# mungerct/Stabilized_Navier_Stokes_Flow_FEniCSx

Hardware: AMD Instinct MI355X
Metric: M-DOF/s (assembly+solve) per Newton iteration (higher is better)
Workload: dtype f64

## Files before the change

### stabilized_navier_stokes_flow_fenicsx_amd/csrc/sns_policy.h

```cpp
#pragma once
#include <algorithm>
#include <cmath>
#include <cstdint>
#include <vector>

#include "sns.h"

namespace sns {
namespace policy {

inline int coarsest_rows(const sns_options& o) { return std::max(o.amg_coarse_size, std::min(o.amg_dense_rows, 4096)); }
inline int small_inverse_rows(const sns_options& o) { return std::max(o.amg_coarse_size, 40); }
enum CoarsestKind { COARSEST_SMALL_INVERSE = 0, COARSEST_BLOCKED_INVERSE = 1, COARSEST_SWEEPS = 2 };
inline CoarsestKind coarsest_kind(const sns_options& o, int64_t rows) {
    if (rows <= small_inverse_rows(o)) return COARSEST_SMALL_INVERSE;
    if (rows <= o.amg_dense_rows) return COARSEST_BLOCKED_INVERSE;
    return COARSEST_SWEEPS;
}
inline bool replicate_from(const sns_options& o, int level, int64_t rows_global, bool fits) {
    return level >= 1 && o.amg_replicate_rows > 0 && rows_global <= (int64_t)o.amg_replicate_rows &&
           rows_global > (int64_t)small_inverse_rows(o) && fits;
}
constexpr int DISTRIBUTED_DENSE_MAX_DOFS = 640;
constexpr int GRAPH_MAX_ROWS = 150000;
// ... 236 lines not shown
enum AssemblyState { STATE_W = 0, STATE_GEXT = 1, STATE_SNAPPED = 2 };
struct AssemblyPlan {
    int error = SNS_OK;
    const char* message = "";
    AssemblyRoute route = ROUTE_STAGED;
    AssemblyState state = STATE_W;
    ElementKernel element = ELEMENT_NONE;
    bool bc_check = false, offdiag = false, diag = false, store_K = false, Fe_out = false, gather_matrix = false,
         gather_residual = false, lift = false, bc_residual = false, matrix = false;
};

inline AssemblyPlan plan_assembly(const AssemblyFacts& f, bool violated = true) {
    AssemblyPlan p;
    auto refuse = [&](const char* why) { p.error = SNS_E_ARG; p.message = why; return p; };
    if (f.form != SNS_FORM_STOKES && f.form != SNS_FORM_NS) return refuse("bad form");
    const bool ns = f.form == SNS_FORM_NS;
    if (ns && !f.has_w) return refuse("NS form needs a state vector");
    p.matrix = f.want_matrix;
    if (f.dim == 2) {
        if (!f.cells) return refuse("empty mesh");
        p.route = ns ? ROUTE_NS_2D : ROUTE_STOKES_2D;
        p.offdiag = f.want_matrix;
        p.diag = f.want_matrix || (!ns && f.has_F);
        if (ns) {
            p.bc_check = f.has_F;
            p.element = f.want_matrix ? ELEMENT_NONE : ELEMENT_RESIDUAL;
            p.Fe_out = p.gather_residual = !f.want_matrix;
            p.lift = f.has_F && violated;
        } else {
            p.state = f.has_w ? STATE_SNAPPED : STATE_GEXT;
            p.bc_residual = f.has_w && f.has_F;
        }
        return p;
    }
    const bool try_fused = f.want_matrix && f.fused && ns && f.cells && !f.variant;
    p.bc_check = ns && f.cells && ((!f.want_matrix && f.has_F) || try_fused);
    const bool fast_residual = p.bc_check && !violated && !f.variant;
    if (try_fused || (!ns && !f.has_w && f.want_matrix && f.fused && f.cells)) {
        p.route = ns ? ROUTE_FUSED_NS : ROUTE_FUSED_STOKES;
        p.state = ns ? STATE_W : STATE_GEXT;
        p.offdiag = p.diag = true;
        p.lift = ns && f.has_F && !fast_residual;
        return p;
    }
    p.element = fast_residual ? ELEMENT_RESIDUAL : f.cells ? ELEMENT_STAGED : ELEMENT_NONE;
    p.store_K = p.element == ELEMENT_STAGED && f.want_matrix;
    p.Fe_out = p.element == ELEMENT_RESIDUAL || (p.element == ELEMENT_STAGED && f.has_F);
    p.gather_matrix = f.want_matrix;
    p.gather_residual = f.has_F;
    return p;
}

struct HandleFacts {
    int dim = 3;
    bool partitioned = false, tt_on = false, vl_on = false, bf_on = false, ev_on = false;
    bool has_facets = false, traction_on = false, backflow_on = false;
};
enum FactBit {
    IS_NOT_3D = 1, IS_PARTITIONED = 2, HAS_TIME_TERM = 4, HAS_LAW = 8, HAS_FORCE = 16, HAS_FIELD = 32, NO_FACETS = 64, HAS_TRACTION = 128,
    HAS_BACKFLOW = 256, HAS_BOUNDARY_FLOW = HAS_TRACTION | HAS_BACKFLOW
};
enum Family { FAMILY_FORM = 0, FAMILY_BOUNDARY, FAMILY_STABILITY, FAMILY_STATE_GRADIENT, FAMILY_RAW_JACOBIAN };
enum FormRequest {
    REQ_SET_TIME_TERM = 0, REQ_CLEAR_TIME_TERM, REQ_SET_CARREAU, REQ_SET_NEWTONIAN, REQ_SET_FIELD ,
    REQ_TIME_STEP, REQ_SHAPE_GRADIENT, REQ_RECOVER_GRADIENT, REQ_ERROR_INDICATOR, REQ_SCALAR ,
    REQ_ELEMENT_VISCOSITY , REQ_FORM_VARIANT, REQ_COUNT
};
enum BoundaryRequest { BREQ_SET_FACETS = 0, BREQ_SET_FLOW, BREQ_SET_SCALAR, BREQ_COUNT };
enum StabilityRequest { SREQ_MASS_APPLY = 0, SREQ_ARNOLDI, SREQ_COUNT, SREQ_MASS_APPLY_TRANSPOSE = SREQ_COUNT, SREQ_ARNOLDI_LEFT, SREQ_KINDS };
constexpr int GREQ_STATE_GRADIENT = 0;
enum RawJacobianRequest { JREQ_APPLY = 0, JREQ_SET_DIRICHLET, JREQ_COUNT };
struct Verdict {
    int error = SNS_OK;
    const char* tail = "";
};
struct Rule {
    Family family;
    int request;
    unsigned any_of;
    int code;
    const char* tail;
};
constexpr Rule RULES[] = {
    {FAMILY_FORM, REQ_SET_TIME_TERM, IS_NOT_3D, SNS_E_ARG, "3-D handles only"},
    {FAMILY_FORM, REQ_SET_TIME_TERM, IS_PARTITIONED, SNS_E_STATE, "not with a communicator attached (partitioned time stepping is not built)"},
    {FAMILY_FORM, REQ_SET_TIME_TERM, HAS_LAW, SNS_E_STATE, "not with a viscosity law set (the transient form has no law)"},
    {FAMILY_FORM, REQ_CLEAR_TIME_TERM, IS_NOT_3D, SNS_E_ARG, "3-D handles only"},
    {FAMILY_FORM, REQ_CLEAR_TIME_TERM, IS_PARTITIONED, SNS_E_STATE, "not with a communicator attached (partitioned time stepping is not built)"},
    {FAMILY_FORM, REQ_SET_CARREAU, IS_NOT_3D, SNS_E_ARG, "3-D handles only"},
    {FAMILY_FORM, REQ_SET_CARREAU, IS_PARTITIONED, SNS_E_STATE, "not with a communicator attached (partitioned handles have no law)"},
    {FAMILY_FORM, REQ_SET_CARREAU, HAS_TIME_TERM, SNS_E_STATE, "not with a time term set (the transient form has no law)"},
    {FAMILY_FORM, REQ_SET_CARREAU, HAS_FORCE | HAS_FIELD, SNS_E_STATE, "not with a body force or a viscosity field set"},
    {FAMILY_FORM, REQ_SET_NEWTONIAN, IS_NOT_3D, SNS_E_ARG, "3-D handles only"},
    {FAMILY_FORM, REQ_SET_NEWTONIAN, IS_PARTITIONED, SNS_E_STATE, "not with a communicator attached (partitioned handles have no law)"},
    {FAMILY_FORM, REQ_SET_NEWTONIAN, HAS_TIME_TERM, SNS_E_STATE, "not with a time term set (the transient form has no law)"},
    {FAMILY_FORM, REQ_SET_FIELD, IS_NOT_3D, SNS_E_ARG, "3-D handles only"},
    {FAMILY_FORM, REQ_SET_FIELD, IS_PARTITIONED, SNS_E_STATE, "not with a communicator attached (partitioned handles have no external fields)"},
    {FAMILY_FORM, REQ_SET_FIELD, HAS_LAW, SNS_E_STATE, "not with a viscosity law set"},
    {FAMILY_FORM, REQ_TIME_STEP, IS_NOT_3D, SNS_E_ARG, "3-D handles only"},
    {FAMILY_FORM, REQ_TIME_STEP, IS_PARTITIONED, SNS_E_STATE, "not with a communicator attached (partitioned time stepping is not built)"},
    {FAMILY_FORM, REQ_TIME_STEP, HAS_LAW, SNS_E_STATE, "not with a viscosity law set (the transient form has no law)"},
    {FAMILY_FORM, REQ_SHAPE_GRADIENT, IS_PARTITIONED, SNS_E_STATE, "not with a communicator attached (partitioned shape gradients are not built)"},
    {FAMILY_FORM, REQ_SHAPE_GRADIENT, HAS_LAW, SNS_E_STATE, "not with a viscosity law set (the mesh derivative of nu_e is not built)"},
    {FAMILY_FORM, REQ_SHAPE_GRADIENT, HAS_FORCE | HAS_FIELD, SNS_E_STATE,
     "not with a body force or a viscosity field set (the mesh derivative is not built with them)"},
    {FAMILY_FORM, REQ_SHAPE_GRADIENT, HAS_BOUNDARY_FLOW, SNS_E_STATE,
     "not with a boundary traction or backflow term set (the mesh derivative of the facet terms is not built)"},
    {FAMILY_FORM, REQ_RECOVER_GRADIENT, IS_PARTITIONED, SNS_E_STATE, "not with a communicator attached (partitioned gradient recovery is not built)"},
    {FAMILY_FORM, REQ_ERROR_INDICATOR, IS_PARTITIONED, SNS_E_STATE,
     "not with a communicator attached (a partitioned indicator needs a halo exchange of G)"},
    {FAMILY_FORM, REQ_SCALAR, IS_NOT_3D, SNS_E_ARG, "3-D handles only"},
    {FAMILY_FORM, REQ_SCALAR, IS_PARTITIONED, SNS_E_STATE, "not with a communicator attached (partitioned scalar transport is not built)"},
    {FAMILY_FORM, REQ_ELEMENT_VISCOSITY, IS_NOT_3D, SNS_E_ARG, "3-D handles only"},
    {FAMILY_FORM, REQ_FORM_VARIANT, IS_NOT_3D, SNS_E_ARG, "3-D handles only"},

    {FAMILY_BOUNDARY, BREQ_SET_FACETS, IS_NOT_3D, SNS_E_ARG, "3-D handles only"},
    {FAMILY_BOUNDARY, BREQ_SET_FACETS, IS_PARTITIONED, SNS_E_STATE, "not with a communicator attached (partitioned boundary terms are not built)"},
    {FAMILY_BOUNDARY, BREQ_SET_FLOW, IS_NOT_3D, SNS_E_ARG, "3-D handles only"},
    {FAMILY_BOUNDARY, BREQ_SET_FLOW, IS_PARTITIONED, SNS_E_STATE, "not with a communicator attached (partitioned boundary terms are not built)"},
    {FAMILY_BOUNDARY, BREQ_SET_FLOW, NO_FACETS, SNS_E_STATE, "set the boundary facets first (sns_set_boundary_facets)"},
    {FAMILY_BOUNDARY, BREQ_SET_SCALAR, IS_NOT_3D, SNS_E_ARG, "3-D handles only"},
    {FAMILY_BOUNDARY, BREQ_SET_SCALAR, IS_PARTITIONED, SNS_E_STATE, "not with a communicator attached (partitioned boundary terms are not built)"},
    {FAMILY_BOUNDARY, BREQ_SET_SCALAR, NO_FACETS, SNS_E_STATE, "set the boundary facets first (sns_set_boundary_facets)"},

    {FAMILY_STABILITY, SREQ_MASS_APPLY, IS_NOT_3D, SNS_E_ARG, "3-D handles only"},
    {FAMILY_STABILITY, SREQ_MASS_APPLY, IS_PARTITIONED, SNS_E_STATE, "not with a communicator attached (partitioned stability analysis is not built)"},
    {FAMILY_STABILITY, SREQ_MASS_APPLY, HAS_LAW, SNS_E_STATE, "not with a viscosity law set (the mass operator of the law's form is not built)"},
    {FAMILY_STABILITY, SREQ_ARNOLDI, IS_NOT_3D, SNS_E_ARG, "3-D handles only"},
    {FAMILY_STABILITY, SREQ_ARNOLDI, IS_PARTITIONED, SNS_E_STATE, "not with a communicator attached (partitioned stability analysis is not built)"},
    {FAMILY_STABILITY, SREQ_ARNOLDI, HAS_LAW, SNS_E_STATE, "not with a viscosity law set (the mass operator of the law's form is not built)"},
    {FAMILY_STABILITY, SREQ_ARNOLDI, HAS_TIME_TERM, SNS_E_STATE, "not with a time term set (the analysis sets its own and clears it)"},

    {FAMILY_STATE_GRADIENT, GREQ_STATE_GRADIENT, IS_NOT_3D, SNS_E_ARG, "3-D handles only"},
    {FAMILY_STATE_GRADIENT, GREQ_STATE_GRADIENT, IS_PARTITIONED, SNS_E_STATE, "not with a communicator attached (the partitioned Hessian pass is not built)"},
    {FAMILY_STATE_GRADIENT, GREQ_STATE_GRADIENT, HAS_LAW, SNS_E_STATE, "not with a viscosity law set (the second derivative of nu_e is not built)"},
    {FAMILY_STATE_GRADIENT, GREQ_STATE_GRADIENT, HAS_TIME_TERM, SNS_E_STATE, "not with a time term set (the pass is taken on the steady form)"},
    {FAMILY_STATE_GRADIENT, GREQ_STATE_GRADIENT, HAS_FORCE, SNS_E_STATE,
     "not with a body force set (J depends on f through the stabilisation's weighting: that contraction is not built)"},
    {FAMILY_STATE_GRADIENT, GREQ_STATE_GRADIENT, HAS_BACKFLOW, SNS_E_STATE,
     "not with a backflow coefficient set (the Hessian of the backflow term is not built)"},

    {FAMILY_RAW_JACOBIAN, JREQ_APPLY, IS_PARTITIONED, SNS_E_STATE, "not with a communicator attached (the partitioned raw-Jacobian pass is not built)"},
    {FAMILY_RAW_JACOBIAN, JREQ_APPLY, HAS_BACKFLOW, SNS_E_STATE,
     "not with a backflow coefficient set (the backflow term's share of the raw Jacobian is not built)"},
    {FAMILY_RAW_JACOBIAN, JREQ_SET_DIRICHLET, IS_PARTITIONED, SNS_E_STATE,
     "not with a communicator attached (partitioned handles keep the Dirichlet values they were created with)"},
};

enum Rows { ROWS_ALL = 0, ROWS_ARG = SNS_E_ARG, ROWS_STATE = SNS_E_STATE };
inline Verdict check_request(Family family, int request, const HandleFacts& f, Rows rows = ROWS_ALL) {
    if (family == FAMILY_STABILITY && request >= SREQ_COUNT) request -= SREQ_COUNT;
    const unsigned facts = (f.dim != 3) * IS_NOT_3D | f.partitioned * IS_PARTITIONED | f.tt_on * HAS_TIME_TERM | f.vl_on * HAS_LAW |
                           f.bf_on * HAS_FORCE | f.ev_on * HAS_FIELD | (!f.has_facets) * NO_FACETS | f.traction_on * HAS_TRACTION |
                           f.backflow_on * HAS_BACKFLOW;
    for (const Rule& r : RULES)
        if (r.family == family && r.request == request && (facts & r.any_of))
            return (rows == ROWS_ALL || r.code == rows) ? Verdict{r.code, r.tail} : Verdict{};
    return {};
}
inline Verdict check_request(Family family, int request, const HandleFacts& f, const Verdict& arguments) {
    Verdict v = check_request(family, request, f, ROWS_ARG);
    if (v.error == SNS_OK) v = arguments;
    if (v.error == SNS_OK) v = check_request(family, request, f, ROWS_STATE);
    return v;
}

constexpr int STABILITY_M_MIN = 2, STABILITY_M_MAX = 64;
struct ArnoldiArgs {
    int m = STABILITY_M_MAX;
    double shift = 0.0, breakdown_rel = 1e-6;
};
inline Verdict check_arnoldi_args(const ArnoldiArgs& a) {
    if (a.m < STABILITY_M_MIN || a.m > STABILITY_M_MAX) return {SNS_E_ARG, "m must lie in [2, 64]"};
    if (!(a.shift >= 0.0) || !(a.shift <= 1.7976931348623157e308)) return {SNS_E_ARG, "the shift must be finite and >= 0"};
    if (!(a.breakdown_rel > 0.0) || !(a.breakdown_rel < 1.0)) return {SNS_E_ARG, "breakdown_rel must lie in (0, 1)"};
    return {};
}
inline Verdict check_arnoldi_extend_args(const ArnoldiArgs& a, int k) {
    const Verdict v = check_arnoldi_args(a);
    if (v.error != SNS_OK) return v;
    if (k < 1 || k > a.m - 1) return {SNS_E_ARG, "k must lie in [1, m - 1]"};
    return {};
}
inline Verdict check_state_gradient_args(double c_jac, double c_mass) {
    if (!(c_jac - c_jac == 0.0) || !(c_mass - c_mass == 0.0)) return {SNS_E_ARG, "the coefficients must be finite"};
    return {};
}

struct RawJacobianArgs {
    int form = SNS_FORM_NS;
    bool aliased = false, variant = false;
};
inline Verdict check_raw_jacobian_args(const RawJacobianArgs& a) {
    if (a.form == SNS_FORM_STOKES) return {SNS_E_ARG, "the Stokes forms are not supported"};
    if (a.form != SNS_FORM_NS) return {SNS_E_ARG, "bad form"};
    if (a.aliased) return {SNS_E_ARG, "x and y must not be the same vector"};
    if (a.variant) return {SNS_E_STATE, "not with a perturbed form variant set (the pass holds the reference's constants only)"};
    return {};
}

inline Verdict check_form_request(FormRequest request, const HandleFacts& f) { return check_request(FAMILY_FORM, request, f); }
inline Verdict check_boundary_request(BoundaryRequest request, const HandleFacts& f) { return check_request(FAMILY_BOUNDARY, request, f); }
inline Verdict check_stability_request(StabilityRequest request, const HandleFacts& f, const ArnoldiArgs& a = {}) {
    const bool arnoldi = request == SREQ_ARNOLDI || request == SREQ_ARNOLDI_LEFT;
    return check_request(FAMILY_STABILITY, request, f, arnoldi ? check_arnoldi_args(a) : Verdict{});
}
inline Verdict check_stability_extend_request(StabilityRequest request, const HandleFacts& f, const ArnoldiArgs& a, int k) {
    return check_request(FAMILY_STABILITY, request, f, check_arnoldi_extend_args(a, k));
}
inline Verdict check_state_gradient_request(const HandleFacts& f, double c_jac = 1.0, double c_mass = 0.0) {
    return check_request(FAMILY_STATE_GRADIENT, GREQ_STATE_GRADIENT, f, check_state_gradient_args(c_jac, c_mass));
}
inline Verdict check_raw_jacobian_request(RawJacobianRequest request, const HandleFacts& f, const RawJacobianArgs& a = {}) {
    return check_request(FAMILY_RAW_JACOBIAN, request, f, request == JREQ_APPLY ? check_raw_jacobian_args(a) : Verdict{});
}

struct FormKey {
    double sigma = 0.0, theta = 0.0;
    bool law_on = false;
    double lambda = 0.0, n = 1.0, r = 0.0;
    uint64_t nu_generation = 0;
    uint64_t boundary_generation = 0;
    bool operator==(const FormKey& o) const {
        return sigma == o.sigma && theta == o.theta && law_on == o.law_on && lambda == o.lambda && n == o.n && r == o.r &&
               nu_generation == o.nu_generation && boundary_generation == o.boundary_generation;
    }
};
struct OperatorKey {
    int form = -1;
    double reynolds = 0.0;
    bool transposed = false;
    FormKey f;
    double scalar[6] = {0, 0, 0, 0, 0, 0};
    bool operator==(const OperatorKey& o) const {
        return form == o.form && reynolds == o.reynolds && transposed == o.transposed && f == o.f &&
               std::equal(scalar, scalar + 6, o.scalar);
    }
};
inline void stamp_operator(OperatorKey& k, int form, double reynolds, const FormKey& f, const double* scalar_par = nullptr) {
    k.form = form;
    k.reynolds = reynolds;
    k.transposed = false;
    k.f = f;
    if (scalar_par) std::copy(scalar_par, scalar_par + 6, k.scalar);
}
inline bool new_operator(const OperatorKey& matrix, const OperatorKey& estimated, bool r3_estimates) {
    return !r3_estimates && !(matrix == estimated);
}

struct LevelDamping {
    double omega = 0.8, lambda_max = 0.0, omega_checked = 0.0, ritz_limit = 0.0;
};
constexpr int ESTIMATE_EVERY = 4;
constexpr double LAMBDA_CAP = 4.0 / 3.0;
constexpr int COMPOUNDING_SWEEPS = 3;
constexpr double GROWTH_BOUND = 0.9;
constexpr double GROWTH_STEP = GROWTH_BOUND;
constexpr int GROWTH_TRIALS = 6;
constexpr double RETRY_FACTOR = 0.7, RETRY_FLOOR = 0.4;

inline bool estimates_due(bool has_estimate, int pc_setups, bool new_operator) {
    return !has_estimate || pc_setups % ESTIMATE_EVERY == 0 || new_operator;
}
inline bool takes_growth_check(bool not_last, int sweeps_per_cycle) { return not_last && sweeps_per_cycle >= COMPOUNDING_SWEEPS; }
inline bool takes_ritz_limit(const sns_options& o, bool not_last, int sweeps_per_cycle) {
    return o.amg_ritz_limit && takes_growth_check(not_last, sweeps_per_cycle);
}
inline double capped_damping(double amg_omega, double backoff, double lambda_max, bool ritz, double ritz_limit) {
    double w = amg_omega * backoff;
    if (lambda_max > 0.0) w = std::min(amg_omega, LAMBDA_CAP / lambda_max) * backoff;
    if (ritz && ritz_limit > 0.0) w = std::min(w, ritz_limit * backoff);
    return w;
}
template <class Growth>
inline int checked_damping(double& w, Growth&& growth) {
    for (int trial = 0; trial < GROWTH_TRIALS; ++trial) {
        double g = 0.0;
        if (const int rc = growth(w, &g)) return rc;
        if (g < GROWTH_BOUND) break;
        w *= GROWTH_STEP;
    }
    return SNS_OK;
}
inline double held_damping(double w, double omega_checked) { return omega_checked > 0.0 ? std::min(w, omega_checked) : w; }
inline bool retryable(int reason) {
    return reason == SNS_KSP_DIVERGED_BREAKDOWN || reason == SNS_KSP_DIVERGED_NANORINF || reason == SNS_KSP_STALLED;
}
inline bool retry_offered(const sns_options& o, double backoff) {
    return o.pc_type == SNS_PC_AMG && o.amg_retry_damping != 0 && backoff > RETRY_FLOOR;
}
inline void back_off(double& backoff) { backoff *= RETRY_FACTOR; }
inline void back_off(LevelDamping& d) {
    d.omega *= RETRY_FACTOR;
    if (d.omega_checked > 0.0) d.omega_checked *= RETRY_FACTOR;
}
inline void forget_estimates(LevelDamping& d) { d.lambda_max = d.omega_checked = d.ritz_limit = 0.0; }

struct StepFacts {
    int nranks = 1, ksp_type = SNS_KSP_BICGSTAB, pc_type = SNS_PC_AMG;
    bool fine_plain_cycle = false, zero_guess_vouched = false, estimates_due = true, plain_step = false;
};
struct StepPlan {
    bool skip_zero_guess_residual = false, export_ax = false, staged_speculation = false, split_cycle = false,
         setup_two_streams = false;
    bool operator==(const StepPlan& o) const {
        return skip_zero_guess_residual == o.skip_zero_guess_residual && export_ax == o.export_ax &&
               staged_speculation == o.staged_speculation && split_cycle == o.split_cycle && setup_two_streams == o.setup_two_streams;
    }
};
inline StepPlan plan_step(const StepFacts& f) {
    StepPlan p;
    if (f.nranks != 1 || f.plain_step || f.ksp_type != SNS_KSP_BICGSTAB) return p;
    p.skip_zero_guess_residual = f.zero_guess_vouched;
    p.export_ax = true;
    p.split_cycle = f.pc_type == SNS_PC_AMG && f.fine_plain_cycle;
    p.staged_speculation = f.pc_type != SNS_PC_AMG || p.split_cycle;
    p.setup_two_streams = f.pc_type == SNS_PC_AMG && !f.estimates_due;
    return p;
}

}
}
```

### stabilized_navier_stokes_flow_fenicsx_amd/csrc/sns_setup.hip

```cpp
#include "sns_ctx.h"

namespace sns {

int alloc_level_vectors(Level& L) {
    const size_t nd = 4 * (size_t)L.n;
    SNS_TRY(L.x.alloc(nd));
    SNS_TRY(L.b.alloc(nd));
    SNS_TRY(L.r.alloc(nd));
    HIP_TRY(hipMemset(L.x, 0, nd * sizeof(double)));
    HIP_TRY(hipMemset(L.b, 0, nd * sizeof(double)));
    HIP_TRY(hipMemset(L.r, 0, nd * sizeof(double)));
    return SNS_OK;
}


int upload_pattern(Level& L, const HostPattern& P, hipStream_t s) {
    L.n = P.n;
    L.nnzb = P.nnzb;
    SNS_TRY(L.rowptr.upload(P.rowptr));
    SNS_TRY(L.colind.upload(P.colind));
    SNS_TRY(L.diag.upload(P.diag));
    SNS_TRY(L.vals.alloc((size_t)P.nnzb * 16));
    SNS_TRY(L.dinv.alloc((size_t)P.n * 16));
    SNS_TRY(L.slot_row.alloc((size_t)P.nnzb));
// ... 379 lines not shown
    const int per_rank_coarse = dist ? std::max(1, o.amg_coarse_size / h->comm->nranks) : o.amg_coarse_size;
    double flag[1] = {n_owned > per_rank_coarse ? 1.0 : 0.0};
    SNS_TRY(global_sum(h, flag, 1));
    more = flag[0] != 0.0 && !(!dist && l >= 1 && n_owned <= policy::coarsest_rows(o));
    return SNS_OK;
}

static int aggregate_level(sns_ctx* h, int l, const Front& f, std::vector<int32_t>& agg, int32_t& nc_owned, int64_t& nc_global,
                           bool& progress) {
    nc_owned = 0;
    if (l == 0 && h->opt.amg_aggregation >= 1) {
        SNS_TRY(aggregate_fine_by_strength(h, f.cur, f.points(), agg, nc_owned));
    } else {
        aggregate_nodes(f.cur, f.n_owned, agg_size(h->opt), agg, nc_owned, f.points());
    }
    if (l == 0) h->agg0 = agg;
    double prog[3] = {(double)f.n_owned, (double)nc_owned, (l == 0 && h->fine_rematched_local) ? 1.0 : 0.0};
    SNS_TRY(global_sum(h, prog, 3));
    if (l == 0) h->fine_rematched = prog[2] > 0.0;
    nc_global = (int64_t)prog[1];
    progress = !(prog[1] >= prog[0] || prog[1] == 0.0);
    if (l == 0 && progress) h->n_global_l1 = nc_global;
    return SNS_OK;
}

static int exchange_aggregate_ids(sns_ctx* h, int l, const Front& f, int32_t nc_owned, std::vector<int32_t>& agg, Plan& cplan,
                                  GhostIds& cghosts, int32_t& nc_total) {
    Comm* c = h->comm.get();
    Level& L = h->levels[l];
    std::vector<double> ids((size_t)4 * f.cur.n, -1.0);
    for (int32_t i = 0; i < f.n_owned; ++i) ids[(size_t)4 * i] = (double)agg[i];
    HIP_TRY(hipMemcpy(L.xg, ids.data(), ids.size() * sizeof(double), hipMemcpyHostToDevice));
    SNS_TRY(comm_exchange(c, c->plans[l], L.xg, h->stream));
    HIP_TRY(hipStreamSynchronize(h->stream));
    HIP_TRY(hipMemcpy(ids.data(), L.xg, ids.size() * sizeof(double), hipMemcpyDeviceToHost));
    HIP_TRY(hipMemset(L.xg, 0, ids.size() * sizeof(double)));
    std::vector<int32_t> owner_agg((size_t)f.cur.n);
    for (int32_t i = 0; i < f.cur.n; ++i) owner_agg[(size_t)i] = (int32_t)ids[(size_t)4 * i];
    return coarse_halo_lists(c->plans[l], owner_agg, nc_owned, agg, cplan, cghosts, nc_total);
}

static int attach_plan(sns_ctx* h, Plan& cplan, int level) {
    SNS_TRY(check_plan_symmetry(h, cplan, level));
    SNS_TRY(plan_upload(cplan));
    SNS_TRY(connect_plan(h, cplan));
    h->comm->plans.push_back(std::move(cplan));
    return SNS_OK;
}

static int flag_empty_aggregates(sns_ctx* h) {
    Level& L = h->levels[0];
    SNS_TRY(L.empty_c.alloc(4 * (size_t)std::max(1, L.nc)));
    if (L.nc > 0)
        hipLaunchKernelGGL(k_empty_coarse, dim3((unsigned)((4 * (int64_t)L.nc + 255) / 256)), dim3(256), 0, h->stream, L.nc, L.m_ptr,
                           L.m_idx, L.free_mask, L.empty_c);
    return SNS_OK;
}

int build_hierarchy(sns_ctx* h, const HostPattern& fine) {
    Comm* c = h->comm.get();
    const bool dist = c && c->active() && c->nranks > 1;
    Front f;
    SNS_TRY(start_front(h, fine, dist, f));
    for (int l = 0; l + 1 < h->opt.amg_max_levels; ++l) {
        bool replicate = false, more = false, progress = false;
        SNS_TRY(agree_replication(h, dist, l, f.n_owned, replicate));
        if (replicate) {
            SNS_TRY(build_replicated_tail(h, l, f));
            return plan_hierarchy(h);
        }
        SNS_TRY(agree_more_levels(h, dist, l, f.n_owned, more));
        if (!more) break;
        std::vector<int32_t> agg;
        int32_t nc_owned = 0;
        int64_t nc_global = 0;
        SNS_TRY(aggregate_level(h, l, f, agg, nc_owned, nc_global, progress));
        if (!progress) break;
        int32_t nc_total = nc_owned;
        Plan cplan;
        GhostIds cghosts;
        if (dist) SNS_TRY(exchange_aggregate_ids(h, l, f, nc_owned, agg, cplan, cghosts, nc_total));
        HostAggregation A;
        build_coarse_from_agg(f.cur, f.n_owned, agg, nc_owned, nc_total, A);
        SNS_TRY(add_next_level(h, l, f, A, nc_global, !dist || l == 0 || c->windows(), dist));
        if (dist) SNS_TRY(attach_plan(h, cplan, l + 1));
        if (l == 0) SNS_TRY(flag_empty_aggregates(h));
        advance(f, A, std::move(cghosts));
    }
    Level& last = h->levels.back();
    if (h->levels.size() > 1) SNS_TRY(dist ? alloc_distributed_coarsest_solver(h, last, f.ghosts) : alloc_coarsest_solver(h, last));
    h->tm.amg_levels = (int)h->levels.size();
    return plan_hierarchy(h);
}


int plan_hierarchy(sns_ctx* h) {
    const Comm* c = h->comm.get();
    const int nl = (int)h->levels.size();
    policy::Facts& f = h->facts;
    f = policy::Facts();
    f.nranks = (c && c->active()) ? std::max(1, c->nranks) : 1;
    f.rep_level = h->rep_level;
    f.rows_global_l1 = h->n_global_l1;
    f.windows = c && c->windows();
    f.team_overlap = h->team_overlap;
    f.fuse_puts = std::getenv("SNS_NO_CARRIED_PUT") == nullptr;
    const Level& last = h->levels.back();
    f.last = last.dense_gj ? policy::COARSEST_BLOCKED_INVERSE
                           : (last.dense_inv || h->cg_N > 0) ? policy::COARSEST_SMALL_INVERSE : policy::COARSEST_SWEEPS;
    f.rep_gather_fits = h->rep_level > 0 && c && c->peer && h->levels[h->rep_level].n_blk > 0 &&
                        (size_t)4 * h->rep_maxn * (size_t)c->nranks <= c->peer->ag_doubles;
    std::vector<double> mine((size_t)2 * nl + 1), all;
    mine[(size_t)2 * nl] = h->fine_rematched_local ? 1.0 : 0.0;
    for (int l = 0; l < nl; ++l) {
        const Level& L = h->levels[l];
        f.rows.push_back(L.n_global);
        f.has_blocks.push_back(L.blk_rows != nullptr);
        f.has_ap.push_back(L.ap_rowptr != nullptr);
        f.has_ap_rep.push_back(L.ap_colind_rep != nullptr);
        const bool wc = c && (size_t)l < c->plans.size() && c->plans[l].identity_recv && c->plans[l].win_recv[0] != nullptr;
        mine[(size_t)l] = wc ? 1.0 : 0.0;
        mine[(size_t)nl + l] = (double)L.n_owned;
    }
    if (f.nranks > 1) SNS_TRY(host_allgather(h, mine, all));
    else all = mine;
    f.win_capable.assign((size_t)nl, 1);
    f.max_owned.assign((size_t)nl, 0);
    for (size_t r = 0; r < all.size() / mine.size(); ++r) {
        if (all[r * mine.size() + 2 * (size_t)nl] != 0.0) f.fine_rematched = true;
        for (int l = 0; l < nl; ++l) {
            if (all[r * mine.size() + l] == 0.0) f.win_capable[(size_t)l] = 0;
            f.max_owned[(size_t)l] = std::max(f.max_owned[(size_t)l], (int64_t)all[r * mine.size() + nl + l]);
        }
    }
    h->plan = policy::plan_cycle(h->opt, f);
    return SNS_OK;
}


static int refresh_replicated_source(sns_ctx* h, const Level& L) {
    Level& C = h->levels[h->rep_level];
    if (L.nnzb > 0)
        HIP_TRY(hipMemcpyAsync(h->rep_vsend, L.vals, (size_t)L.nnzb * 16 * sizeof(double), hipMemcpyDeviceToDevice, h->stream));
    SNS_TRY(comm_allgather(h->comm.get(), h->rep_vsend, h->rep_vrecv, (int)(h->rep_maxnz * 16), h->stream));
    const int64_t nsrc = h->rep_maxnz * h->comm->nranks;
    hipLaunchKernelGGL(k_scatter_blocks, dim3((unsigned)((nsrc * 8 + 255) / 256)), dim3(256), 0, h->stream, nsrc, h->rep_valmap,
                       h->rep_vrecv, C.vals);
    return SNS_OK;
}

static int refresh_smoother_inverses(sns_ctx* h, const policy::LevelPlan& P, Level& L) {
    const int32_t rows = L.n_owned;
    if (rows > 0) hipLaunchKernelGGL(k_dinv, dim3((rows + 255) / 256), dim3(256), 0, h->stream, rows, L.diag, L.vals, L.dinv);
    if (!P.blocks) return SNS_OK;
    const int bf = h->opt.amg_f32_matrix == 2 ? 2 : 1;
    if (!L.binv32 || L.binv_fmt != bf) {
        SNS_TRY(L.binv32.alloc(binv_bytes_per_block(bf) * (size_t)std::max(1, L.n_blk)));
        L.binv_fmt = bf;
    }
    if (L.n_blk > 0)
        with_fmt(bf, [&](auto F) {
            hipLaunchKernelGGL((k_binv<F>), dim3((unsigned)((L.n_blk + 7) / 8)), dim3(256), 0, h->stream, L.n_blk, L.blk_rows,
                               L.blk_of, L.rowptr, L.colind, L.vals, L.binv32, h->d_sing);
        });
    return SNS_OK;
}

static int refresh_low_precision_copies(sns_ctx* h, const policy::LevelPlan& P, Level& L, bool not_last) {
    if (P.lp_fmt == 0) return SNS_OK;
    const int32_t rows = L.n_owned;
    if (!L.dinv32) SNS_TRY(L.dinv32.alloc((size_t)16 * std::max(1, L.n)));
    if (rows > 0)
        hipLaunchKernelGGL(k_cvt_f32, dim3(vec_grid(16 * (int64_t)rows)), dim3(256), 0, h->stream, 16 * (int64_t)rows, L.dinv,
                           L.dinv32);
    if (h->opt.amg_f32_matrix == 2) {
        if (!L.vals16) {
            SNS_TRY(L.vals16.alloc(std::max<size_t>(1, (size_t)L.nnzb * 4) * sizeof(uint2)));
            SNS_TRY(L.scale16.alloc((size_t)4 * std::max(1, L.n)));
        }
        const bool with_m = not_last && L.ap_rowptr && L.ap_nib && h->opt.amg_fused_post;
        if (with_m && !L.ap_vals16) {
            SNS_TRY(L.ap_vals16.alloc(std::max<size_t>(1, (size_t)L.ap_nnz * 4) * sizeof(uint2)));
            SNS_TRY(L.ap_scale16.alloc((size_t)4 * std::max(1, L.n)));
        }
        if (rows > 0) {
            const unsigned grid = (unsigned)((rows + 31) / 32);
            if (with_m)
                hipLaunchKernelGGL((k_lp_copies16<1>), dim3(grid), dim3(128), 0, h->stream, rows, L.rowptr, L.vals,
                                   (uint2*)L.vals16.get(), L.scale16, L.ap_rowptr, L.ap_colind, L.ap_ptr, L.ap_idx, L.ap_nib, L.agg,
                                   L.free_mask, (uint2*)L.ap_vals16.get(), L.ap_scale16);
            else
                hipLaunchKernelGGL((k_lp_copies16<0>), dim3(grid), dim3(128), 0, h->stream, rows, L.rowptr, L.vals,
                                   (uint2*)L.vals16.get(), L.scale16, (const int32_t*)nullptr, (const int32_t*)nullptr,
                                   (const int32_t*)nullptr, (const int32_t*)nullptr, (const uint64_t*)nullptr,
                                   (const int32_t*)nullptr, (const uint8_t*)nullptr, (uint2*)nullptr, (float*)nullptr);
        }
    }
    if (h->opt.amg_f32_matrix != 2) {
        if (!L.vals32) SNS_TRY(L.vals32.alloc((size_t)L.nnzb * 16));
        if (L.nnzb > 0)
            hipLaunchKernelGGL(k_cvt_f32, dim3(vec_grid(L.nnzb * 16)), dim3(256), 0, h->stream, L.nnzb * 16, L.vals, L.vals32);
    }
    return SNS_OK;
}

static int refresh_ap32(sns_ctx* h, const policy::LevelPlan& P, Level& L) {
    if (!(L.ap_rowptr && h->opt.amg_fused_post && P.lp_fmt == 1)) return SNS_OK;
    const int32_t rows = L.n_owned;
    if (!L.ap_vals32) SNS_TRY(L.ap_vals32.alloc((size_t)L.ap_nnz * 16));
    if (rows > 0)
        hipLaunchKernelGGL(k_ap_cvt32, dim3((unsigned)((4 * (int64_t)rows + 255) / 256)), dim3(256), 0, h->stream, rows,
                           L.ap_rowptr, L.ap_colind, L.ap_ptr, L.ap_idx, L.vals, L.agg, L.free_mask, (float4*)L.ap_vals32.get());
    return SNS_OK;
}

static void refresh_galerkin(sns_ctx* h, int l) {
    const Level& L = h->levels[l];
    Level& C = h->levels[l + 1];
    const int64_t nth = C.nnzb * 8;
    hipLaunchKernelGGL(k_galerkin, dim3((unsigned)((nth + 255) / 256)), dim3(256), 0, h->stream, C.nnzb, L.r_ptr, L.r_idx, L.vals,
                       C.slot_row, C.colind, (l == 0) ? L.empty_c.get() : (const uint8_t*)nullptr, L.m_ptr, C.vals);
}

static int refresh_coarsest_solver(sns_ctx* h, int l) {
    Level& L = h->levels[l];
    if (h->cg_N > 0) {
        const int N = h->cg_N, mr = 4 * h->cg_maxn;
        HIP_TRY(hipMemsetAsync(h->cg_rows, 0, (size_t)mr * N * sizeof(double), h->stream));
        const int64_t nth = L.nnzb * 16;
        if (nth > 0)
            hipLaunchKernelGGL(k_bsr_to_dense_map, dim3((unsigned)((nth + 255) / 256)), dim3(256), 0, h->stream, L.n_owned,
                               L.rowptr, L.colind, L.vals, h->cg_colmap, N, h->cg_rows);
        hipLaunchKernelGGL(k_pad_identity, dim3(1), dim3(256), 0, h->stream, 4 * L.n_owned, mr, h->comm->rank * mr, N, h->cg_rows);
        SNS_TRY(comm_allgather(h->comm.get(), h->cg_rows, h->cg_full, mr * N, h->stream));
        hipLaunchKernelGGL(k_dense_inverse, dim3(1), dim3(1024), 0, h->stream, N, h->cg_full, h->d_piv, h->d_sing);
    } else if (L.dense_gj) {
        const int N = 4 * L.n, Np = L.dense_np;
        HIP_TRY(hipMemsetAsync(L.dense_gj, 0, (size_t)Np * Np * sizeof(double), h->stream));
        const int64_t nth = L.nnzb * 16;
        hipLaunchKernelGGL(k_bsr_to_dense_ld, dim3((unsigned)((nth + 255) / 256)), dim3(256), 0, h->stream, L.nnzb, L.slot_row,
                           L.colind, L.vals, Np, L.dense_gj);
        if (Np > N) hipLaunchKernelGGL(k_dense_pad_diag, dim3((Np - N + 255) / 256), dim3(256), 0, h->stream, N, Np, L.dense_gj);
        if (!h->gj_stream && std::getenv("SNS_GJ_TWO_STREAMS") &&
            hipStreamCreateWithFlags(h->gj_stream.put(), hipStreamNonBlocking) != hipSuccess) h->gj_stream.reset();
        dense_gj_inverse(h->stream, h->gj_stream, Np, L.dense_gj, L.dense_work, h->d_sing);
        const int64_t nn = (int64_t)Np * Np;
        hipLaunchKernelGGL(k_dense_to_f32, dim3((unsigned)((nn / 4 + 255) / 256)), dim3(256), 0, h->stream, nn, L.dense_gj, L.dense_x32);
    } else if (L.dense_inv) {
        const int N = 4 * L.n;
        HIP_TRY(hipMemsetAsync(L.dense_inv, 0, (size_t)N * N * sizeof(double), h->stream));
        const int64_t nth = L.nnzb * 16;
        hipLaunchKernelGGL(k_bsr_to_dense, dim3((unsigned)((nth + 255) / 256)), dim3(256), 0, h->stream, L.n, L.rowptr, L.colind,
                           L.vals, L.dense_inv);
        hipLaunchKernelGGL(k_dense_inverse, dim3(1), dim3(1024), 0, h->stream, N, L.dense_inv, h->d_piv, h->d_sing);
    }
    return SNS_OK;
}

static int conclude_setup(sns_ctx* h, int nl, bool check_sing, int sing) {
    if (check_sing) {
        double bad[1] = {sing != 0 ? 1.0 : 0.0};
        SNS_TRY(global_sum(h, bad, 1));
        if (bad[0] != 0.0) {
            HIP_TRY(hipMemset(h->d_sing, 0, sizeof(int)));
            set_error("AMG setup: a dense inverse (coarsest level or an aggregate block" +
                      std::string(sing != 0 ? "" : ", on another rank") + ") met a zero or non-finite pivot; set "
                      "amg_dense_rows = 0 / amg_block_smooth = 0");
            return SNS_E_STATE;
        }
    }
    if (h->comm && h->comm->peer && h->opt.pc_type == SNS_PC_AMG)
        for (int l = 0; l < nl && l < (int)h->comm->plans.size(); ++l) {
            const Level& L = h->levels[l];
            if (L.blk_rows && L.n_blk > 0 && L.binv32)
                SNS_TRY(comm_plan_put_groups(h->comm.get(), h->comm->plans[l], L.blk_rows, 8 * L.n_blk, h->stream));
        }
    return SNS_OK;
}


static int setup_chain_ready(sns_ctx* h, int nl) {
    if (!h->setup_stream) {
        int least = 0, greatest = 0;
        HIP_TRY(hipDeviceGetStreamPriorityRange(&least, &greatest));
        HIP_TRY(hipStreamCreateWithPriority(h->setup_stream.put(), hipStreamNonBlocking, greatest));
        HIP_TRY(hipEventCreateWithFlags(h->ev_setup_fork.put(), hipEventDisableTiming));
        HIP_TRY(hipEventCreateWithFlags(h->ev_setup_join.put(), hipEventDisableTiming));
    }
    while ((int)h->ev_setup_level.size() < nl) {
        h->ev_setup_level.emplace_back();
        HIP_TRY(hipEventCreateWithFlags(h->ev_setup_level.back().put(), hipEventDisableTiming));
    }
    return SNS_OK;
}

int pc_setup(sns_ctx* h) {
    if (!h->has_matrix) { set_error("pc_setup before a matrix was assembled"); return SNS_E_STATE; }
    HIP_TRY(hipEventRecord(h->ev0, h->stream));
    const int nl = (h->opt.pc_type == SNS_PC_AMG) ? (int)h->levels.size() : 1;
    bool any_block = false;
    const bool new_operator = policy::new_operator(h->matrix_key, h->est_key, h->r3_estimates);
    bool estimates_due = false;
    for (int l = 0; l < nl; ++l) estimates_due = estimates_due || damping_estimates_due(h, l, nl, new_operator);
    const bool two = step_plan(h, false, estimates_due).setup_two_streams;
    hipStream_t const user = h->stream;
    struct OnChain {
        sns_ctx* h;
        hipStream_t user;
        OnChain(sns_ctx* hh, bool two) : h(hh), user(hh->stream) { if (two) h->stream = h->setup_stream; }
        ~OnChain() { h->stream = user; }
    };
    if (two) {
        SNS_TRY(setup_chain_ready(h, nl));
        HIP_TRY(hipEventRecord(h->ev_setup_fork, user));
        HIP_TRY(hipStreamWaitEvent(h->setup_stream, h->ev_setup_fork, 0));
    }
    for (int l = 0; l < nl; ++l) {
        Level& L = h->levels[l];
        if (h->rep_level > 0 && l == h->rep_level - 1) {
            SNS_TRY(refresh_replicated_source(h, L));
            continue;
        }
        const policy::LevelPlan& P = h->plan.level[(size_t)l];
        const bool not_last = l + 1 < nl;
        if (two && l >= 1) HIP_TRY(hipStreamWaitEvent(user, h->ev_setup_level[(size_t)l], 0));
        SNS_TRY(refresh_smoother_inverses(h, P, L));
        if (P.blocks) any_block = true;
        SNS_TRY(refresh_low_precision_copies(h, P, L, not_last));
        SNS_TRY(damping_decide(h, l, nl, new_operator));
        if (not_last) {
            SNS_TRY(refresh_ap32(h, P, L));
            OnChain chain(h, two);
            refresh_galerkin(h, l);
            if (two) HIP_TRY(hipEventRecord(h->ev_setup_level[(size_t)l + 1], h->setup_stream));
        } else if (nl > 1) {
            OnChain chain(h, two);
            SNS_TRY(refresh_coarsest_solver(h, l));
        }
    }
    if (two) {
        HIP_TRY(hipEventRecord(h->ev_setup_join, h->setup_stream));
        HIP_TRY(hipStreamWaitEvent(user, h->ev_setup_join, 0));
    }
    if (const char* miss = plan_buffer_missing(h)) {
        set_error(std::string("AMG setup: the cycle's plan needs ") + miss + ", which the setup did not allocate");
        return SNS_E_STATE;
    }
    ++h->pc_setups;
    h->est_key = h->matrix_key;
    const bool check_sing = nl > 1 && (h->levels[nl - 1].dense_gj != nullptr || any_block);
    int* h_sing = reinterpret_cast<int*>(h->h_scal + 768);
    *h_sing = 0;
    if (check_sing) HIP_TRY(hipMemcpyAsync(h_sing, h->d_sing, sizeof(int), hipMemcpyDeviceToHost, h->stream));
    HIP_TRY(hipEventRecord(h->ev1, h->stream));
    HIP_TRY(hipStreamSynchronize(h->stream));
    float ms = 0;
    HIP_TRY(hipEventElapsedTime(&ms, h->ev0, h->ev1));
    h->tm.pc_setup_ms += ms;
    HIP_TRY(hipGetLastError());
    SNS_TRY(conclude_setup(h, nl, check_sing, *h_sing));
    h->pc_ready = true;
    return SNS_OK;
}


const char* plan_buffer_missing(const sns_ctx* h) {
    if (h->opt.pc_type != SNS_PC_AMG) return nullptr;
    for (size_t l = 0; l < h->plan.level.size() && l < h->levels.size(); ++l) {
        const policy::LevelPlan& P = h->plan.level[l];
        const Level& L = h->levels[l];
        if (P.blocks && (!L.binv32 || L.binv_fmt != (P.lp_fmt == 2 ? 2 : 1))) return "a level's aggregate-block inverses";
        if (P.lp_fmt != 0 && (!L.dinv32 || !(P.lp_fmt == 2 ? (const void*)L.vals16 : (const void*)L.vals32)))
            return "a level's low-precision matrix copy";
        if (P.fused_post && !(P.lp_fmt == 2 ? (const void*)L.ap_vals16 : (const void*)L.ap_vals32)) return "a level's M = A P";
    }
    return nullptr;
}


int get_vec(sns_ctx* h, size_t k, double** out) {
    while (h->kv.size() <= k) {
        DevBuf<double> p;
        SNS_TRY(p.alloc((size_t)ld_of(h)));
        HIP_TRY(hipMemset(p, 0, (size_t)ld_of(h) * sizeof(double)));
        h->kv.push_back(std::move(p));
    }
    *out = h->kv[k];
    return SNS_OK;
}

}
```

Before: 53.40.

## Issue whole Galerkin chain on setup stream up front, overlapping smoother estimates

The full chain of Galerkin coarse-operator products and the coarsest solver refresh is now enqueued on a separate setup stream before the per-level smoother/damping work begins. The user stream waits on per-level events before using each level. Two-stream setup is also enabled when damping estimates are due, unless a replicated level exists. This is meant to let the host-synchronising eigenvalue estimates run alongside the Galerkin products instead of serialising with them. It adds a scope guard that joins the setup stream on early exit, and it risks ordering problems if the Galerkin chain depends on state refreshed in the per-level loop.

```diff
diff --git a/stabilized_navier_stokes_flow_fenicsx_amd/csrc/sns_policy.h b/stabilized_navier_stokes_flow_fenicsx_amd/csrc/sns_policy.h
--- a/stabilized_navier_stokes_flow_fenicsx_amd/csrc/sns_policy.h
+++ b/stabilized_navier_stokes_flow_fenicsx_amd/csrc/sns_policy.h
@@ -562,10 +562,11 @@
 };
 struct StepPlan {
     bool skip_zero_guess_residual = false, export_ax = false, staged_speculation = false, split_cycle = false,
-         setup_two_streams = false;
+         setup_two_streams = false, setup_chain_beside_estimates = false;
     bool operator==(const StepPlan& o) const {
         return skip_zero_guess_residual == o.skip_zero_guess_residual && export_ax == o.export_ax &&
-               staged_speculation == o.staged_speculation && split_cycle == o.split_cycle && setup_two_streams == o.setup_two_streams;
+               staged_speculation == o.staged_speculation && split_cycle == o.split_cycle &&
+               setup_two_streams == o.setup_two_streams && setup_chain_beside_estimates == o.setup_chain_beside_estimates;
     }
 };
 inline StepPlan plan_step(const StepFacts& f) {
@@ -576,6 +577,7 @@
     p.split_cycle = f.pc_type == SNS_PC_AMG && f.fine_plain_cycle;
     p.staged_speculation = f.pc_type != SNS_PC_AMG || p.split_cycle;
     p.setup_two_streams = f.pc_type == SNS_PC_AMG && !f.estimates_due;
+    p.setup_chain_beside_estimates = f.pc_type == SNS_PC_AMG && f.estimates_due;
     return p;
 }
 
diff --git a/stabilized_navier_stokes_flow_fenicsx_amd/csrc/sns_setup.hip b/stabilized_navier_stokes_flow_fenicsx_amd/csrc/sns_setup.hip
--- a/stabilized_navier_stokes_flow_fenicsx_amd/csrc/sns_setup.hip
+++ b/stabilized_navier_stokes_flow_fenicsx_amd/csrc/sns_setup.hip
@@ -705,18 +705,33 @@
     const bool new_operator = policy::new_operator(h->matrix_key, h->est_key, h->r3_estimates);
     bool estimates_due = false;
     for (int l = 0; l < nl; ++l) estimates_due = estimates_due || damping_estimates_due(h, l, nl, new_operator);
-    const bool two = step_plan(h, false, estimates_due).setup_two_streams;
+    const policy::StepPlan plan = step_plan(h, false, estimates_due);
+    const bool two = (plan.setup_two_streams || plan.setup_chain_beside_estimates) && h->rep_level == 0;
     hipStream_t const user = h->stream;
     struct OnChain {
         sns_ctx* h;
         hipStream_t user;
-        OnChain(sns_ctx* hh, bool two) : h(hh), user(hh->stream) { if (two) h->stream = h->setup_stream; }
+        explicit OnChain(sns_ctx* hh) : h(hh), user(hh->stream) { h->stream = h->setup_stream; }
         ~OnChain() { h->stream = user; }
     };
+    struct JoinChain {
+        sns_ctx* h;
+        hipStream_t user;
+        bool open = false;
+        ~JoinChain() { if (open) (void)hipStreamWaitEvent(user, h->ev_setup_join, 0); }
+    } join{h, user};
     if (two) {
         SNS_TRY(setup_chain_ready(h, nl));
         HIP_TRY(hipEventRecord(h->ev_setup_fork, user));
         HIP_TRY(hipStreamWaitEvent(h->setup_stream, h->ev_setup_fork, 0));
+        OnChain chain(h);
+        for (int l = 0; l + 1 < nl; ++l) {
+            refresh_galerkin(h, l);
+            HIP_TRY(hipEventRecord(h->ev_setup_level[(size_t)l + 1], h->setup_stream));
+        }
+        if (nl > 1) SNS_TRY(refresh_coarsest_solver(h, nl - 1));
+        HIP_TRY(hipEventRecord(h->ev_setup_join, h->setup_stream));
+        join.open = true;
     }
     for (int l = 0; l < nl; ++l) {
         Level& L = h->levels[l];
@@ -733,16 +748,13 @@
         SNS_TRY(damping_decide(h, l, nl, new_operator));
         if (not_last) {
             SNS_TRY(refresh_ap32(h, P, L));
-            OnChain chain(h, two);
-            refresh_galerkin(h, l);
-            if (two) HIP_TRY(hipEventRecord(h->ev_setup_level[(size_t)l + 1], h->setup_stream));
-        } else if (nl > 1) {
-            OnChain chain(h, two);
+            if (!two) refresh_galerkin(h, l);
+        } else if (nl > 1 && !two) {
             SNS_TRY(refresh_coarsest_solver(h, l));
         }
     }
     if (two) {
-        HIP_TRY(hipEventRecord(h->ev_setup_join, h->setup_stream));
+        join.open = false;
         HIP_TRY(hipStreamWaitEvent(user, h->ev_setup_join, 0));
     }
     if (const char* miss = plan_buffer_missing(h)) {
```

After: 53.35. No clear change (-0.1%).
